# Hippogriff/parsenet-codebase

Measured on AMD Instinct MI355X. Metric: shapes/sec fwd+bwd on 10k-pt clouds, higher is better.
Workload: dtype f32; 1 GPU; cfg5: ParSeNet e2e (seg + mean-shift 10 it. + per-segment spline/primitive fit + Chamfer/residual), 10k pts, batch 4 per GPU, fwd+bwd+allreduce+Adam; batch_per_gpu=4, points=10000, k=80, parallelism=dp1, global_batch=4

## Files before the change

parsenet_codebase_amd/csrc/knn.hip:

```cpp
#include "knn_common.h"

__global__ void pn_knn_sqnorm_kernel(const float* __restrict__ x, int C, int N, int c0, int c1,
                                     float* __restrict__ xx, const int* __restrict__ gate_any) {
  const int b = blockIdx.y;
  if (gate_any && !gate_any[b]) return;
  const int j = blockIdx.x * blockDim.x + threadIdx.x;
  if (j >= N) return;
  const float* xb = x + (size_t)b * C * N;
  float acc = 0.f;
  for (int c = c0; c < c1; ++c) {
    float v = xb[(size_t)c * N + j];
    acc = __builtin_fmaf(v, v, acc);
  }
  xx[(size_t)b * N + j] = acc;
}

template <int MODE, bool TAIL>
__device__ static inline void knn_tile(const float* __restrict__ xb, const float* __restrict__ xxb,
                                       int C, int Nend, int j0, int qc, int N, float xxq,
                                       float tau, int& cnt, u64* __restrict__ mylist) {
  float acc[KNN_TC];
  float accn[MODE == 1 ? KNN_TC : 1];
#pragma unroll
  for (int t = 0; t < KNN_TC; ++t) acc[t] = 0.f;
// ... 43 lines not shown
    const bool ok = TAIL ? (j0 + t < Nend) : true;
    if (ok && v >= tau) {
      mylist[cnt] = knn_key(v, j0 + t);
      ++cnt;
    }
  }
}

template <int MODE>
__global__ __launch_bounds__(256) void pn_knn_scan_kernel(const float* __restrict__ x,
                                                          const float* __restrict__ xx, int C,
                                                          int N, int k, int S, int slice_len,
                                                          u64* __restrict__ lists,
                                                          int* __restrict__ counts,
                                                          KnnIdxOut out,
                                                          const int* __restrict__ gate) {
  __shared__ __attribute__((aligned(16))) uint32_t s_hist[4][256];
  const int b = blockIdx.z;
  const int slice = blockIdx.y;
  const int wave = threadIdx.x >> 6, lane = threadIdx.x & 63;
  const int qbase = (blockIdx.x * 4 + wave) * 64;
  if (qbase >= N) return;
  const int q = qbase + lane;
  const bool qvalid = q < N;
  const int qc = qvalid ? q : N - 1;
  const int Np = (N + 63) & ~63;
  if (gate && !__any(qvalid && gate[(size_t)b * N + qc] != 0)) return;
  const float* __restrict__ xb = x + (size_t)b * C * N;
  const float* __restrict__ xxb = xx + (size_t)b * N;
  u64* __restrict__ wlists = lists + (((size_t)b * Np + qbase) * S + slice) * KNN_CAP;
  const size_t lstride = (size_t)S * KNN_CAP;
  u64* __restrict__ mylist = wlists + (size_t)lane * lstride;
  uint32_t* hist = s_hist[wave];
// ... 98 lines not shown
  *slice_len_out = len;
}

size_t pn_knn_v1_workspace(int B, int C, int N, int k, bool gated) {
  (void)C;
  int S, len;
  knn_plan(B, N, k, gated, &S, &len);
  const size_t Np = pn_align_up(N, 64);
  return pn_align_up((size_t)B * N * sizeof(float), 256) +
         pn_align_up((size_t)B * Np * S * sizeof(int), 256) +
         pn_align_up((size_t)B * Np * S * KNN_CAP * sizeof(u64), 256);
}

int pn_knn_v1_launch(int mode, const float* x, int B, int C, int N, int k, KnnIdxOut idx,
                     void* workspace, size_t workspace_bytes, hipStream_t stream,
                     const int* gate, const int* gate_any) {
  PN_CHECK_ARG(x && idx.p, "pn_knn: null pointer");
  PN_CHECK_ARG(B > 0 && C > 0 && N > 0, "pn_knn: empty input (B=%d C=%d N=%d)", B, C, N);
  PN_CHECK_ARG(k >= 1 && k <= KNN_MAXK, "pn_knn: k=%d unsupported (1..%d)", k, KNN_MAXK);
  PN_CHECK_ARG(k <= N, "pn_knn: k=%d exceeds the number of points N=%d", k, N);
  PN_CHECK_ARG(mode == 0 || C == 6, "pn_knn_pn: points+normals metric needs C=6, got %d", C);
  PN_CHECK_ARG(workspace && workspace_bytes >= pn_knn_v1_workspace(B, C, N, k, gate != nullptr),
               "pn_knn: workspace too small");
  int S, slice_len;
  knn_plan(B, N, k, gate != nullptr, &S, &slice_len);
  const size_t Np = pn_align_up(N, 64);
  char* w = (char*)workspace;
  float* xx = (float*)w;
  w += pn_align_up((size_t)B * N * sizeof(float), 256);
  int* counts = (int*)w;
  w += pn_align_up((size_t)B * Np * S * sizeof(int), 256);
  u64* lists = (u64*)w;
  dim3 g1(pn_cdiv(N, 256), B);
  hipLaunchKernelGGL(pn_knn_sqnorm_kernel, g1, dim3(256), 0, stream, x, C, N, 0,
                     mode == 0 ? C : 3, xx, gate ? gate_any : nullptr);
  PN_CHECK_LAUNCH();
  dim3 grid(pn_cdiv(N, 256), S, B);
  PN_PROF(gate ? "knn_scan_gated" : "knn_scan", stream);
  if (mode == 0)
    hipLaunchKernelGGL(pn_knn_scan_kernel<0>, grid, dim3(256), 0, stream, x, xx, C, N, k, S,
                       slice_len, lists, counts, idx, gate);
  else
    hipLaunchKernelGGL(pn_knn_scan_kernel<1>, grid, dim3(256), 0, stream, x, xx, C, N, k, S,
                       slice_len, lists, counts, idx, gate);
  PN_CHECK_LAUNCH();
  if (S > 1) {
    const long long nq = (long long)B * N;
    hipLaunchKernelGGL(pn_knn_merge_kernel, dim3(pn_cdiv(nq, 4)), dim3(256), 0, stream, lists,
                       counts, N, k, S, nq, idx);
    PN_CHECK_LAUNCH();
  }
  return PN_OK;
}
```

parsenet_codebase_amd/csrc/knn_common.h:

```cpp
#pragma once
#include "common.h"

#define KNN_TC 32
#define KNN_CAP 1024
#define KNN_CAP0 256
#define KNN_MAXK 128
#define KNN_EPL (KNN_CAP / 64)

typedef unsigned long long u64;

struct KnnIdxOut {
  void* p;
  int is32;
  __host__ __device__ explicit operator bool() const { return p != nullptr; }
  __device__ inline void put(size_t pos, int64_t v) const {
    if (is32)
      static_cast<int*>(p)[pos] = (int)v;
    else
      static_cast<int64_t*>(p)[pos] = v;
  }
};

__device__ static inline u64 knn_key(float v, int j) {
  if (v == 0.0f) v = 0.0f;
  return ((u64)pn_f2ord(v) << 32) | (u64)(0xffffffffu - (uint32_t)j);
}
__device__ static inline int64_t knn_key_index(u64 key) {
  return key ? (int64_t)(0xffffffffu - (uint32_t)(key & 0xffffffffu)) : 0;
}

__device__ static inline u64 readlane_u64(u64 v, int l) {
  uint32_t lo = __builtin_amdgcn_readlane((uint32_t)v, l);
  uint32_t hi = __builtin_amdgcn_readlane((uint32_t)(v >> 32), l);
  return ((u64)hi << 32) | lo;
}

__device__ static u64 knn_wave_select_ge(u64* __restrict__ lp, int n, int k, uint32_t* __restrict__ hist,
                                         float slack, int* __restrict__ kept) {
  const int lane = threadIdx.x & 63;
  u64 key[KNN_EPL];
#pragma unroll
  for (int e = 0; e < KNN_EPL; ++e) {
    int s = e * 64 + lane;
// ... 113 lines not shown
```

parsenet_codebase_amd/csrc/knn_mfma.hip:

```cpp
#include "knn_common.h"
#include "split_common.h"

typedef float f32x16 __attribute__((ext_vector_type(16)));

size_t pn_knn_v1_workspace(int B, int C, int N, int k, bool gated);
int pn_knn_v1_launch(int mode, const float* x, int B, int C, int N, int k, KnnIdxOut idx,
                     void* workspace, size_t workspace_bytes, hipStream_t stream,
                     const int* gate, const int* gate_any = nullptr);

struct KnnPerm {
  uint32_t a, c, mask;
  int n;
};

__host__ __device__ static inline int knn_perm(const KnnPerm& p, int i) {
  uint32_t v = (uint32_t)i;
  do {
    v = (v * p.a + p.c) & p.mask;
  } while (v >= (uint32_t)p.n);
  return (int)v;
}

static KnnPerm knn_make_perm(int N, bool identity) {
  KnnPerm p;
  int m = 1;
  while ((1u << m) < (uint32_t)N) ++m;
  p.mask = (m >= 32) ? 0xffffffffu : ((1u << m) - 1u);
  p.a = identity ? 1u : (((uint32_t)(0.6180339887498949 * (double)(1ull << m))) | 1u);
  p.c = identity ? 0u : ((0x9E3779B9u >> (32 - m)) | 1u);
  p.n = N;
  return p;
}

__global__ void pn_knn_prep_kernel(const float* __restrict__ x, int C, int N, int Cp, int Np,
                                   int mode, int point_major, KnnPerm perm,
                                   float* __restrict__ xp, float* __restrict__ xxp) {
  const int b = blockIdx.y;
  const int jp = blockIdx.x * blockDim.x + threadIdx.x;
  if (jp >= Np) return;
  const float* xb = x + (size_t)b * C * N;
  float* xpb = xp + (size_t)b * Cp * Np;
  float acc = 0.f;
  if (jp < N) {
    const int j = knn_perm(perm, jp);
    const int cnorm = mode == 1 ? 3 : C;
    int c = 0;
    for (; c + 8 <= C; c += 8) {
      float v[8];
#pragma unroll
      for (int e = 0; e < 8; ++e) v[e] = point_major ? xb[(size_t)j * C + c + e] : xb[(size_t)(c + e) * N + j];
#pragma unroll
      for (int e = 0; e < 8; ++e) {
        const int cd = (mode == 1 && c + e >= 3) ? c + e + 1 : c + e;
        xpb[(size_t)cd * Np + jp] = v[e];
        if (c + e < cnorm) acc = __builtin_fmaf(v[e], v[e], acc);
      }
    }
    for (; c < C; ++c) {
      const float v = point_major ? xb[(size_t)j * C + c] : xb[(size_t)c * N + j];
      const int cd = (mode == 1 && c >= 3) ? c + 1 : c;
      xpb[(size_t)cd * Np + jp] = v;
      if (c < cnorm) acc = __builtin_fmaf(v, v, acc);
    }
    if (mode == 1) {
      xpb[(size_t)3 * Np + jp] = 0.f;
      xpb[(size_t)7 * Np + jp] = 0.f;
    } else {
      for (int c = C; c < Cp; ++c) xpb[(size_t)c * Np + jp] = 0.f;
    }
  } else {
    for (int c = 0; c < Cp; ++c) xpb[(size_t)c * Np + jp] = 0.f;
  }
  xxp[(size_t)b * Np + jp] = acc;
}

__global__ __launch_bounds__(256) void pn_knn_prep_pm_kernel(const float* __restrict__ x, int C, int N,
                                                            int Cp, int Np, KnnPerm perm,
                                                            float* __restrict__ xp,
                                                            float* __restrict__ xxp) {
  extern __shared__ float prep_tile[];
  const int b = blockIdx.y;
  const int jp0 = blockIdx.x * 64;
  const int t = threadIdx.x;
  const float* xb = x + (size_t)b * C * N;
// ... 13 lines not shown
  const int p = t & 63, part = t >> 6;
  if (jp0 + p < Np) {
    for (int c = part; c < Cp; c += 4) xpb[(size_t)c * Np + jp0 + p] = c < C ? prep_tile[p * ld + c] : 0.f;
    if (part == 0) {
      float acc = 0.f;
      for (int c = 0; c < C; ++c) {
        const float v = prep_tile[p * ld + c];
        acc = __builtin_fmaf(v, v, acc);
      }
      xxp[(size_t)b * Np + jp0 + p] = acc;
    }
  }
}

static void knn_prep_launch(hipStream_t stream, const float* x, int B, int C, int N, int Cp, int Np, int mode,
                            int point_major, KnnPerm perm, float* xp, float* xxp) {
  if (point_major && mode != 1 && (C & 3) == 0 && C <= 224) {
    hipLaunchKernelGGL(pn_knn_prep_pm_kernel, dim3(pn_cdiv(Np, 64), B), dim3(256), 64 * (C + 1) * sizeof(float),
                       stream, x, C, N, Cp, Np, perm, xp, xxp);
  } else {
    hipLaunchKernelGGL(pn_knn_prep_kernel, dim3(pn_cdiv(Np, 64), B), dim3(64), 0, stream, x, C, N, Cp, Np,
                       mode, point_major, perm, xp, xxp);
  }
}

template <int KSTEPS, int QSETS, int MODE, int KIND>
__global__ __launch_bounds__(256) void pn_knn_mfma_kernel(
    const float* __restrict__ xq, const float* __restrict__ xxq_, int Nq, int Nqp,
    const float* __restrict__ xc, const float* __restrict__ xxc_, int Nc, int Ncp,
    int tiles_per_slice, float* __restrict__ tilemax, const float* __restrict__ tau,
    u64* __restrict__ lists, int* __restrict__ counts, int subcap, KnnPerm perm_c) {
  constexpr bool COLLECT = KIND == 1;
  constexpr bool ARGMAX = KIND == 2;
  constexpr int CP = 2 * KSTEPS;
  constexpr int TILE = CP * 32;
  __shared__ __attribute__((aligned(16))) float lds[2][TILE + 32];
  const int b = blockIdx.z;
// ... 153 lines not shown

__global__ void pn_knn_argmax_final_kernel(const u64* __restrict__ lists, int Nq, int Nqp, int S,
                                           KnnPerm perm_q, KnnIdxOut out_idx) {
  const int b = blockIdx.y;
  const int qp = blockIdx.x * blockDim.x + threadIdx.x;
  if (qp >= Nq) return;
  const u64* l = lists + ((size_t)b * Nqp + qp) * S * 2;
  u64 best = 0;
  for (int i = 0; i < 2 * S; ++i) best = l[i] > best ? l[i] : best;
  out_idx.put((size_t)b * Nq + knn_perm(perm_q, qp), knn_key_index(best));
}

#define KM_TR 16
__global__ __launch_bounds__(256) void pn_knn_tau_kernel(const float* __restrict__ tilemax, int Nq,
                                                         int Nqp, int T, int k,
                                                         float* __restrict__ tau) {
  const int b = blockIdx.y;
  const int wave = threadIdx.x >> 6, lane = threadIdx.x & 63;
  const int q = blockIdx.x * 4 + wave;
  if (q >= Nq) return;
  const float* __restrict__ row = tilemax + ((size_t)b * Nqp + q) * T;
  float v[KM_TR];
  float vmin = __builtin_inff(), vmax = -__builtin_inff();
#pragma unroll
  for (int e = 0; e < KM_TR; ++e) {
    const int t = e * 64 + lane;
    v[e] = t < T ? row[t] : -__builtin_inff();
    if (v[e] > -__builtin_inff()) vmin = fminf(vmin, v[e]);
    vmax = fmaxf(vmax, v[e]);
  }
  for (int t = KM_TR * 64 + lane; t < T; t += 64) {
// ... 14 lines not shown
    const float fm = pn_ord2f(mid);
    int c = 0;
#pragma unroll
    for (int e = 0; e < KM_TR; ++e) c += __builtin_popcountll(__ballot(v[e] >= fm));
    for (int t0 = KM_TR * 64; t0 < T; t0 += 64) {
      const int t = t0 + lane;
      c += __builtin_popcountll(__ballot(t < T && row[t] >= fm));
    }
    if (c >= k) {
      lo = mid;
      if (c <= k + slack) break;
    } else {
      hi = mid;
    }
  }
  if (lane == 0) tau[(size_t)b * Nqp + q] = pn_ord2f(lo);
}

__global__ __launch_bounds__(256) void pn_knn_final_kernel(
    const u64* __restrict__ lists, const int* __restrict__ counts, int Nq, int Nqp, int k, int S,
    int subcap, KnnPerm perm_q, KnnPerm perm_c, KnnIdxOut out_idx,
    float* __restrict__ out_val, int* __restrict__ flags, int* __restrict__ anyflag) {
  __shared__ __attribute__((aligned(16))) uint32_t s_hist[4][256];
  __shared__ u64 s_keys[4][KNN_CAP];
  const int b = blockIdx.y;
  const int wave = threadIdx.x >> 6, lane = threadIdx.x & 63;
  const int qp = blockIdx.x * 4 + wave;
  if (qp >= Nq) return;
  const size_t ql = (size_t)b * Nqp + qp;
  const int qo = knn_perm(perm_q, qp);
  u64* keys = s_keys[wave];
  const int nsub = 2 * S;
// ... 202 lines not shown
  if (kind == 0)
    hipLaunchKernelGGL((pn_knn_mfma_kernel<KSTEPS, QSETS, MODE, 0>), grid, dim3(256), 0, stream, xq,
                       xxq, Nq, Nqp, xc, xxc, Nc, Ncp, tps, tilemax, tau, lists, cnt, subcap, perm_c);
  else if (kind == 1)
    hipLaunchKernelGGL((pn_knn_mfma_kernel<KSTEPS, QSETS, MODE, 1>), grid, dim3(256), 0, stream, xq,
                       xxq, Nq, Nqp, xc, xxc, Nc, Ncp, tps, tilemax, tau, lists, cnt, subcap, perm_c);
  else if (MODE == 2)
    hipLaunchKernelGGL((pn_knn_mfma_kernel<KSTEPS, QSETS, MODE, (MODE == 2 ? 2 : 0)>), grid,
                       dim3(256), 0, stream, xq, xxq, Nq, Nqp, xc, xxc, Nc, Ncp, tps, tilemax, tau,
                       lists, cnt, subcap, perm_c);
}

static int select_run(const KnnPlan& p, const KnnWs& w, int mode, bool self, const float* q,
                      int q_pm, int Nq, const float* c, int c_pm, int Nc, int B, int C, int k,
                      KnnIdxOut out_idx, float* out_val, int* flags_out, char* base,
                      hipStream_t stream, bool approx_value = false) {
  float* xc = (float*)(base + w.xc);
  float* xxc = (float*)(base + w.xxc);
  float* xq = (float*)(base + w.xq);
  float* xxq = (float*)(base + w.xxq);
  float* tilemax = (float*)(base + w.tilemax);
  float* tau = (float*)(base + w.tau);
  int* cnt = (int*)(base + w.cnt);
  int* flags = flags_out ? flags_out : (int*)(base + w.flags);
  int* anyflag = flags_out ? nullptr : flags + (size_t)B * Nq;
  u64* lists = (u64*)(base + w.lists);
  const bool argmax = mode == 2 && k == 1 && out_val == nullptr && out_idx.p != nullptr && !self;
  const KnnPerm perm_c = knn_make_perm(Nc, argmax);
  const KnnPerm perm_q = self ? perm_c : knn_make_perm(Nq, true);

  PN_CHECK_HIP(hipMemsetAsync(flags, 0, ((size_t)B * Nq + (flags_out ? 0 : B)) * 4, stream));
  {
    PN_PROF("knn_prep", stream);
    knn_prep_launch(stream, c, B, C, Nc, p.Cp, p.Ncp, mode, c_pm, perm_c, xc, xxc);
    if (!self) knn_prep_launch(stream, q, B, C, Nq, p.Cp, p.Nqp, mode, q_pm, perm_q, xq, xxq);
  }
  PN_CHECK_LAUNCH();
  const bool x3p1 = !argmax && (approx_value ? knn_x3_pass1(p, 0, true) : knn_x3_pass1(p, mode));
  if (approx_value && !(x3p1 && mode == 2 && out_val && !out_idx.p)) {
    pn_set_error("select_run: the bf16 x 3 value selection needs C <= 128 and Nc >= 2048");
    return PN_ERR_UNSUPPORTED;
  }
  const bool x3p2 = x3p1 && knn_x3_level() >= 2 && self && mode == 0 && out_idx.p && !out_val;
  u32x4* img = (u32x4*)(base + w.img);
  unsigned* xxmax = (unsigned*)(base + w.xxmax);
  float* xpm = x3p2 ? (float*)(base + w.xpm) : nullptr;
  float* xxo = x3p2 ? (float*)(base + w.xxo) : nullptr;
  const float x3A = 4.0f * (float)(p.Cp + 2) * 0x1p-24f;
  const bool centre = x3p2 && knn_x3_centre();
  const float x3Ao = centre ? (float)(p.Cp + 4) * 0x1p-24f : 0.f;
  const int np1 = knn_x3_p1_products(mode, centre);
  const float x3A1 = np1 == 3 ? x3A + 3.1f * 0x1p-16f : x3A;
  const int np2 = (centre && np1 == 3 && getenv("PN_KNN_X3_P2") && atoi(getenv("PN_KNN_X3_P2")) == 3) ? 3 : 6;
  const float x3A2 = np2 == 3 ? x3A1 : x3A;
  float* mu = centre ? (float*)(base + w.mu) : nullptr;
  float* xpc = centre ? (float*)(base + w.xpc) : nullptr;
  float* xxcc = centre ? (float*)(base + w.xxcc) : nullptr;
  float* xxoc = centre ? (float*)(base + w.xxoc) : nullptr;
  unsigned* xxmaxc = centre ? (unsigned*)(base + w.xxmaxc) : nullptr;
  if (x3p1) {
    PN_PROF("knn_x3_image", stream);
    PN_CHECK_HIP(hipMemsetAsync(xxmax, 0, (size_t)B * 8, stream));
    if (centre) {
      hipLaunchKernelGGL(pn_knn_x3_mean_kernel, dim3(p.Cp, B), dim3(256), 0, stream, (const float*)xc, p.Cp, p.Ncp, Nc, mu);
    }
    dim3 ig(p.Ncp / 32, B);
    if (p.ksteps == 32)
      hipLaunchKernelGGL(pn_knn_x3_image_kernel<8>, ig, dim3(256), 0, stream, xc, xxc, p.Ncp, img, xxmax, Nc, perm_c,
                         xpm, xxo, (const float*)mu, xpc, xxcc, xxoc, xxmaxc);
    else if (p.ksteps == 64)
      hipLaunchKernelGGL(pn_knn_x3_image_kernel<16>, ig, dim3(256), 0, stream, xc, xxc, p.Ncp, img, xxmax, Nc, perm_c,
                         xpm, xxo, (const float*)mu, xpc, xxcc, xxoc, xxmaxc);
    else
      hipLaunchKernelGGL(pn_knn_x3_image_kernel<32>, ig, dim3(256), 0, stream, xc, xxc, p.Ncp, img, xxmax, Nc, perm_c,
                         xpm, xxo, (const float*)mu, xpc, xxcc, xxoc, xxmaxc);
    PN_CHECK_LAUNCH();
  }
  const float* xq_a = centre ? (const float*)xpc : (const float*)xq;
  const float* xxq_a = centre ? (const float*)xxcc : (const float*)xxq;
  const float* xxc_a = centre ? (const float*)xxcc : (const float*)xxc;
  const unsigned* xxmax_a = centre ? (const unsigned*)xxmaxc : (const unsigned*)xxmax;
  if (p.fused && x3p2) {
    const char* ne = getenv("PN_KNN_FUSED_NP");
    const int npf = (ne && atoi(ne) == 6) ? 6 : 3;
    const float Af = npf == 3 ? x3A + 3.1f * 0x1p-16f : x3A;
    const int qpw = 128 * p.qsets, ntiles = p.Ncp / 32, subcapf = KNN_CAP / 2;
    dim3 gf(1, pn_cdiv(p.Nqp, qpw), B);
    {
      PN_PROF(p.ksteps == 32 ? "knn_x3_fused_c64" : "knn_x3_fused_wide", stream);
#define KX_GOF(NCH, QS, TPS_, NP_)                                                                                       \
// ... 60 lines not shown
  }
        if (mode == 0 && p.ksteps == 32)
          KX_GO1(8, 2, 0, 2)
        else if (mode == 0 && p.ksteps == 64)
          KX_GO1(16, 1, 0, 1)
        else if (mode == 0)
          KX_GO1(32, 1, 0, 1)
        else if (p.ksteps == 32)
          KX_GO1(8, 2, 2, 2)
        else
          KX_GO1(16, 1, 2, 1)
      }
      PN_CHECK_LAUNCH();
      {
        PN_PROF("knn_tau", stream);
        hipLaunchKernelGGL(pn_knn_tau_kernel, dim3(pn_cdiv(Nq, 4), B), dim3(256), 0, stream,
                           tilemax, Nq, p.Nqp, p.Ncp / 16, k, tau);
        if (!approx_value || np1 == 3)
          hipLaunchKernelGGL(pn_knn_x3_margin_kernel, dim3(pn_cdiv(Nq, 256), B), dim3(256), 0, stream, tau, xxq_a, Nq,
                             p.Nqp, xxmax_a, x3p2 ? x3A2 : x3A, mode, (x3p2 || approx_value) ? 2.0f : 1.0f, x3A1,
                             (const float*)xxq, (const unsigned*)xxmax, x3Ao);
      }
      PN_CHECK_LAUNCH();
      if (approx_value) {
        int tpsv = tps1;
        if (pn_cdiv(ntiles, tpsv) > KX_MAX_SLICES) tpsv = (int)pn_align_up(pn_cdiv(ntiles, KX_MAX_SLICES), 2);
        const int Sv = pn_cdiv(ntiles, tpsv);
        int subcapv = (int)pn_align_up(3 * k / (2 * Sv) + 16, 8);
        if (2 * Sv * subcapv > 2 * p.S * p.subcap) subcapv = (2 * p.S * p.subcap) / (2 * Sv);
        if (2 * Sv * subcapv > KNN_CAP) subcapv = KNN_CAP / (2 * Sv);
        dim3 gv(Sv, pn_cdiv(p.Nqp, qpw), B);
        {
          PN_PROF("sel_x3_pass2_dot", stream);
          if (p.ksteps == 32)
            KX_GO(8, 2, 2, 2, 1, gv, tpsv, subcapv);
          else
// ... 82 lines not shown
        KM_GO(2, 2, 0);
      else if (p.ksteps == 4)
        KM_GO(4, 2, 0);
      else if (p.ksteps == 32)
        KM_GO(32, 2, 0);
      else if (p.ksteps == 64)
        KM_GO(64, 1, 0);
      else
        KM_GO(128, 1, 0);
#undef KM_GO
    }
    PN_CHECK_LAUNCH();
    if (collect == 0) {
      PN_PROF("knn_tau", stream);
      hipLaunchKernelGGL(pn_knn_tau_kernel, dim3(pn_cdiv(Nq, 4), B), dim3(256), 0, stream,
                         tilemax, Nq, p.Nqp, p.Ncp / 16, k, tau);
      PN_CHECK_LAUNCH();
    }
  }
  if (argmax) {
    PN_PROF("knn_final", stream);
    hipLaunchKernelGGL(pn_knn_argmax_final_kernel, dim3(pn_cdiv(Nq, 256), B), dim3(256), 0, stream, lists,
                       Nq, p.Nqp, p.S, perm_q, out_idx);
    PN_CHECK_LAUNCH();
    return PN_OK;
  }
  {
    PN_PROF("knn_final", stream);
    hipLaunchKernelGGL(pn_knn_final_kernel, dim3(pn_cdiv(Nq, 4), B), dim3(256), 0, stream, lists,
                       cnt, Nq, p.Nqp, k, p.S, p.subcap, perm_q, perm_c, out_idx, out_val, flags, anyflag);
  }
// ... 145 lines not shown
  const int tps = pn_cdiv(ntiles, S);
  S = pn_cdiv(ntiles, tps);
  int subcap = (int)pn_align_up(3 * k / (2 * S) + 16, 8);
  if (2 * S * subcap > 2 * p.S * p.subcap) subcap = (2 * p.S * p.subcap) / (2 * S);
  if (2 * S * subcap > KNN_CAP) subcap = KNN_CAP / (2 * S);
  dim3 grid(S, pn_cdiv(Nq, 256), B);
  {
    PN_PROF("sel_h2_pass1_dot", stream);
    hipLaunchKernelGGL(pn_dotsel_h2_kernel<0>, grid, dim3(512), 0, stream, q, Nq, p.Nqp, (const u32x4*)img_c,
                       Nc, p.Ncp, tps, tilemax, (const float*)tau, lists, cnt, subcap);
  }
  PN_CHECK_LAUNCH();
  {
    PN_PROF("knn_tau", stream);
    hipLaunchKernelGGL(pn_knn_tau_kernel, dim3(pn_cdiv(Nq, 4), B), dim3(256), 0, stream, tilemax, Nq, p.Nqp,
                       p.Ncp / 16, k, tau);
  }
  PN_CHECK_LAUNCH();
  {
    PN_PROF("sel_h2_pass2_dot", stream);
    hipLaunchKernelGGL(pn_dotsel_h2_kernel<1>, grid, dim3(512), 0, stream, q, Nq, p.Nqp, (const u32x4*)img_c,
                       Nc, p.Ncp, tps, tilemax, (const float*)tau, lists, cnt, subcap);
  }
  PN_CHECK_LAUNCH();
  {
    PN_PROF("knn_final", stream);
    hipLaunchKernelGGL(pn_knn_final_kernel, dim3(pn_cdiv(Nq, 4), B), dim3(256), 0, stream, lists, cnt, Nq,
                       p.Nqp, k, S, subcap, ident_q, ident_c, KnnIdxOut{nullptr, 0}, out_val, flags, (int*)nullptr);
  }
  PN_CHECK_LAUNCH();
  return PN_OK;
// ... 24 lines not shown
  PN_CHECK_ARG(k >= 1 && k <= KNN_MAXK, "pn_knn: k=%d unsupported (1..%d)", k, KNN_MAXK);
  PN_CHECK_ARG(k <= N, "pn_knn: k=%d exceeds the number of points N=%d", k, N);
  PN_CHECK_ARG(mode == 0 || C == 6, "pn_knn_pn: points+normals metric needs C=6, got %d", C);
  PN_CHECK_ARG(workspace && workspace_bytes >= pn_knn_workspace(B, C, N, k),
               "pn_knn: workspace too small");
  const KnnPlan p = knn_mfma_plan(mode, B, C, N, N, k, false);
  if (!(p.fused && knn_x3_level() >= 2)) {
    const KskPlan sk = ksk_plan(mode, B, C, N, k);
    if (sk.ok) return ksk_run(sk, x, B, C, N, k, idx.p, idx.is32, (char*)workspace, stream);
  }
  if (!p.fast)
    return pn_knn_v1_launch(mode, x, B, C, N, k, idx, workspace, workspace_bytes, stream, nullptr);
  const KnnWs w = knn_mfma_ws(p, B, C, N, k, true, true);
  char* base = (char*)workspace;
  int rc = select_run(p, w, mode, true, x, 0, N, x, 0, N, B, C, k, idx, nullptr, nullptr, base,
                      stream);
  if (rc) return rc;
  PN_PROF("knn_fallback_gate", stream);
  return pn_knn_v1_launch(mode, x, B, C, N, k, idx, base + w.v1,
                          pn_knn_v1_workspace(B, C, N, k, true), stream, (int*)(base + w.flags),
                          (int*)(base + w.flags) + (size_t)B * N);
}

extern "C" int pn_knn_f32(const float* x, int B, int C, int N, int k, int64_t* idx,
                          void* workspace, size_t workspace_bytes, void* stream) {
  return knn_dispatch(0, x, B, C, N, k, KnnIdxOut{idx, 0}, workspace, workspace_bytes, (hipStream_t)stream);
}

extern "C" int pn_knn_pn_f32(const float* x6, int B, int N, int k, int64_t* idx, void* workspace,
                             size_t workspace_bytes, void* stream) {
  return knn_dispatch(1, x6, B, 6, N, k, KnnIdxOut{idx, 0}, workspace, workspace_bytes, (hipStream_t)stream);
}

extern "C" int pn_knn_graph_i32(const float* x, int B, int C, int N, int k, int metric, int32_t* idx,
                                void* workspace, size_t workspace_bytes, void* stream) {
  PN_CHECK_ARG(metric == 0 || metric == 1, "pn_knn_graph_i32: metric %d", metric);
// ... 28 lines not shown
```

parsenet_codebase_amd/csrc/knn_x3.h:

```cpp
#pragma once

template <int NCH>
__host__ __device__ static inline int knx_slot(int r, int q) {
  return r * NCH + (q ^ (NCH == 8 ? ((r >> 1) & 7) : x3_swz(r)));
}

__global__ __launch_bounds__(256) void pn_knn_x3_mean_kernel(const float* __restrict__ xp, int CP, int Np, int N,
                                                             float* __restrict__ mu) {
  __shared__ float red[256];
  const int c = blockIdx.x, b = blockIdx.y, t = threadIdx.x;
  const float* row = xp + ((size_t)b * CP + c) * Np;
  float acc = 0.f;
  for (int j = t; j < N; j += 256) acc += row[j];
  red[t] = acc;
  __syncthreads();
#pragma unroll
  for (int o = 128; o > 0; o >>= 1) {
    if (t < o) red[t] += red[t + o];
    __syncthreads();
  }
  if (t == 0) mu[(size_t)b * CP + c] = red[0] / (float)N;
}

template <int NCH>
__global__ __launch_bounds__(256) void pn_knn_x3_image_kernel(const float* __restrict__ xp,
                                                              const float* __restrict__ xxp, int Np,
                                                              u32x4* __restrict__ img,
                                                              unsigned* __restrict__ xxmax, int N, KnnPerm perm,
                                                              float* __restrict__ xpm, float* __restrict__ xxo,
                                                              const float* __restrict__ mu, float* __restrict__ xpc,
                                                              float* __restrict__ xxcc, float* __restrict__ xxoc,
                                                              unsigned* __restrict__ xxmaxc) {
  constexpr int CP = 8 * NCH;
  __shared__ double s_part[8][32][2];
  const int b = blockIdx.y, t = blockIdx.x, tid = threadIdx.x;
  const int r = tid & 31;
  const float* src = xp + (size_t)b * CP * Np + (size_t)t * 32 + r;
  u32x4* dst = img + ((size_t)b * (Np / 32) + t) * (3 * 32 * NCH);
  const int jp = t * 32 + r;
  const int jo = (xpm && jp < N) ? knn_perm(perm, jp) : -1;
  double part_mx = 0.0, part_mm = 0.0;
  for (int q = tid >> 5; q < NCH; q += 8) {
    float v[8];
#pragma unroll
    for (int e = 0; e < 8; ++e) v[e] = src[(size_t)(8 * q + e) * Np];
    if (jo >= 0) {
      float4* d = reinterpret_cast<float4*>(xpm + ((size_t)b * N + jo) * CP + 8 * q);
      d[0] = make_float4(v[0], v[1], v[2], v[3]);
      d[1] = make_float4(v[4], v[5], v[6], v[7]);
    }
    if (mu) {
#pragma unroll
      for (int e = 0; e < 8; ++e) {
        const float m = mu[(size_t)b * CP + 8 * q + e];
        part_mx = __builtin_fma((double)m, (double)v[e], part_mx);
        part_mm = __builtin_fma((double)m, (double)m, part_mm);
        v[e] = jp < N ? v[e] - m : 0.f;
        xpc[((size_t)b * CP + 8 * q + e) * Np + jp] = v[e];
      }
    }
    u32x4 vh, vm, vl;
    X3_SPLIT_TO(v[0], v[1], vh, vm, vl, 0);
    X3_SPLIT_TO(v[2], v[3], vh, vm, vl, 1);
    X3_SPLIT_TO(v[4], v[5], vh, vm, vl, 2);
    X3_SPLIT_TO(v[6], v[7], vh, vm, vl, 3);
    const int slot = knx_slot<NCH>(r, q);
    dst[slot] = vh;
    dst[32 * NCH + slot] = vm;
    dst[2 * 32 * NCH + slot] = vl;
  }
  if (mu) {
    s_part[tid >> 5][r][0] = part_mx;
    s_part[tid >> 5][r][1] = part_mm;
    __syncthreads();
  }
  if (tid < 64) {
    const float nrm = tid < 32 ? xxp[(size_t)b * Np + (size_t)t * 32 + tid] : 0.f;
    if (tid < 32 && jo >= 0) xxo[(size_t)b * N + jo] = nrm;
    const float m = pn_wave_max(nrm);
    if (tid == 0) atomicMax(&xxmax[b], __float_as_uint(fmaxf(m, 0.f)));
    if (mu) {
      float nc = 0.f;
      if (tid < 32) {
        double mx = 0.0, mm = 0.0;
#pragma unroll
        for (int g = 0; g < 8; ++g) {
          mx += s_part[g][tid][0];
          mm += s_part[g][tid][1];
        }
        nc = jp < N ? (float)(((double)nrm - 2.0 * mx) + mm) : 0.f;
        xxcc[(size_t)b * Np + (size_t)t * 32 + tid] = nc;
        if (jo >= 0) xxoc[(size_t)b * N + jo] = nc;
      }
      const float mc = pn_wave_max(nc);
      if (tid == 0) atomicMax(&xxmaxc[b], __float_as_uint(fmaxf(mc, 0.f)));
    }
  }
}

__device__ static inline float knx_eps(float nq, float nc, float A, int mode) {
  nq = fmaxf(nq, 0.f);
  nc = fmaxf(nc, 0.f);
  const float cross = sqrtf(nq * nc) * 1.000001f;
  return (mode == 0 ? 2.0f * A * cross + 0x1p-21f * (nq + nc) : A * cross) * 1.0001f;
}

#define KX_NW 4
#define KX_WPE(NCH, MODE) ((NCH) == 32 ? 1 : ((NCH) == 16 && (MODE) == 2 ? 3 : 2))
template <int NCH, int QSETS, int MODE, int TPS, int KIND, int NP = 6>
__global__ __launch_bounds__(64 * KX_NW) __attribute__((amdgpu_waves_per_eu(KX_WPE(NCH, MODE), KX_WPE(NCH, MODE)))) void pn_knn_x3_pass_kernel(
    const float* __restrict__ xq, const float* __restrict__ xxq_, int Nq, int Nqp,
    const u32x4* __restrict__ PC, const float* __restrict__ xxc_, int Nc, int Ncp, int tiles_per_slice,
    float* __restrict__ tilemax, const float* __restrict__ tau, u64* __restrict__ lists,
    int* __restrict__ counts, int subcap, const unsigned* __restrict__ xxmax,
    const float* __restrict__ xxq_o = nullptr, const unsigned* __restrict__ xxmax_o = nullptr, float A_ = 0.f,
    float Ao_ = 0.f) {
  static_assert(KIND != 2 || MODE == 0, "the fused form is built for the squared-distance metric");
  constexpr int CP = 8 * NCH, KS = NCH / 2, PIECE = 32 * NCH, IMG = 3 * PIECE;
  constexpr int CHUNKS = TPS * IMG / 64;
  static_assert(CHUNKS % KX_NW == 0 && (TPS == 1 || TPS == 2 || TPS == 4), "chunks are dealt evenly to the waves");
// ... 241 lines not shown
      }
    }
    cur ^= 1;
  }
#undef KX_STAGE
  if (KIND >= 1 && wave_on) {
#pragma unroll
    for (int u = 0; u < QSETS; ++u) {
      const int q = q0 + 32 * u + col;
      if (q < Nqp) counts[(((size_t)b * Nqp + q) * gridDim.x + slice) * 2 + h] = mycnt[u];
    }
  }
}


__global__ void pn_knn_x3_margin_kernel(float* __restrict__ tau, const float* __restrict__ xxq, int Nq, int Nqp,
                                        const unsigned* __restrict__ xxmax, float A, int mode, float times, float A1,
                                        const float* __restrict__ xxq_o, const unsigned* __restrict__ xxmax_o, float Ao) {
  const int b = blockIdx.y;
  const int q = blockIdx.x * blockDim.x + threadIdx.x;
  if (q >= Nq) return;
  const float nq = xxq[(size_t)b * Nqp + q], nc = __uint_as_float(xxmax[b]);
  float eps = knx_eps(nq, nc, A1, mode) + (times - 1.0f) * knx_eps(nq, nc, A, mode);
  if (Ao > 0.f) eps += times * knx_eps(xxq_o[(size_t)b * Nqp + q], __uint_as_float(xxmax_o[b]), Ao, mode);
  const float t = tau[(size_t)b * Nqp + q];
  tau[(size_t)b * Nqp + q] = t - eps - 0x1p-22f * fabsf(t);
}

template <int CP>
__device__ static inline float knx_exact_dot(const float* __restrict__ xq, const float* __restrict__ xcrow) {
  constexpr int CB = CP > 128 ? 128 : CP;
  float dot = 0.f;
#pragma clang loop unroll(disable)
  for (int c0 = 0; c0 < CP; c0 += CB) {
    const float4* xc = reinterpret_cast<const float4*>(xcrow + c0);
    float4 cv[CB / 4];
#pragma unroll
    for (int c4 = 0; c4 < CB / 4; ++c4) cv[c4] = xc[c4];
#pragma unroll
    for (int c4 = 0; c4 < CB / 4; ++c4) {
      const float4 qv = *reinterpret_cast<const float4*>(xq + c0 + 4 * c4);
      dot = __builtin_fmaf(qv.x, cv[c4].x, dot);
      dot = __builtin_fmaf(qv.y, cv[c4].y, dot);
// ... 145 lines not shown
```

Baseline: 178.5 shapes/s.

## Fuse KNN prep, mean, margin and flag-clear kernels; reuse norms in fallback

Merges several small KNN launches. The centred x3 path now reads the source directly in a combined mean and prep kernel, and zeroing of flags and maxima moves into the prep kernels, which drops memsets. The tau margin is folded into the tau kernel. The v1 fallback reuses squared norms written by prep and exits early for batches with no gated points. This trims launch and memory-pass overhead, but the new prep kernel recomputes norms from shared memory and reads strided source data, and the fallback's correctness now depends on xx being written in prep.

Result: no change. 178.0 shapes/s (-0.3%).

```diff
diff --git a/parsenet_codebase_amd/csrc/knn.hip b/parsenet_codebase_amd/csrc/knn.hip
--- a/parsenet_codebase_amd/csrc/knn.hip
+++ b/parsenet_codebase_amd/csrc/knn.hip
@@ -81,9 +81,11 @@
                                                           u64* __restrict__ lists,
                                                           int* __restrict__ counts,
                                                           KnnIdxOut out,
-                                                          const int* __restrict__ gate) {
+                                                          const int* __restrict__ gate,
+                                                          const int* __restrict__ gate_any) {
   __shared__ __attribute__((aligned(16))) uint32_t s_hist[4][256];
   const int b = blockIdx.z;
+  if (gate_any && !gate_any[b]) return;
   const int slice = blockIdx.y;
   const int wave = threadIdx.x >> 6, lane = threadIdx.x & 63;
   const int qbase = (blockIdx.x * 4 + wave) * 64;
@@ -212,7 +214,7 @@
 
 int pn_knn_v1_launch(int mode, const float* x, int B, int C, int N, int k, KnnIdxOut idx,
                      void* workspace, size_t workspace_bytes, hipStream_t stream,
-                     const int* gate, const int* gate_any) {
+                     const int* gate, const int* gate_any, bool xx_ready) {
   PN_CHECK_ARG(x && idx.p, "pn_knn: null pointer");
   PN_CHECK_ARG(B > 0 && C > 0 && N > 0, "pn_knn: empty input (B=%d C=%d N=%d)", B, C, N);
   PN_CHECK_ARG(k >= 1 && k <= KNN_MAXK, "pn_knn: k=%d unsupported (1..%d)", k, KNN_MAXK);
@@ -229,18 +231,20 @@
   int* counts = (int*)w;
   w += pn_align_up((size_t)B * Np * S * sizeof(int), 256);
   u64* lists = (u64*)w;
-  dim3 g1(pn_cdiv(N, 256), B);
-  hipLaunchKernelGGL(pn_knn_sqnorm_kernel, g1, dim3(256), 0, stream, x, C, N, 0,
-                     mode == 0 ? C : 3, xx, gate ? gate_any : nullptr);
-  PN_CHECK_LAUNCH();
+  if (!xx_ready) {
+    dim3 g1(pn_cdiv(N, 256), B);
+    hipLaunchKernelGGL(pn_knn_sqnorm_kernel, g1, dim3(256), 0, stream, x, C, N, 0,
+                       mode == 0 ? C : 3, xx, gate ? gate_any : nullptr);
+    PN_CHECK_LAUNCH();
+  }
   dim3 grid(pn_cdiv(N, 256), S, B);
   PN_PROF(gate ? "knn_scan_gated" : "knn_scan", stream);
   if (mode == 0)
     hipLaunchKernelGGL(pn_knn_scan_kernel<0>, grid, dim3(256), 0, stream, x, xx, C, N, k, S,
-                       slice_len, lists, counts, idx, gate);
+                       slice_len, lists, counts, idx, gate, gate ? gate_any : nullptr);
   else
     hipLaunchKernelGGL(pn_knn_scan_kernel<1>, grid, dim3(256), 0, stream, x, xx, C, N, k, S,
-                       slice_len, lists, counts, idx, gate);
+                       slice_len, lists, counts, idx, gate, gate ? gate_any : nullptr);
   PN_CHECK_LAUNCH();
   if (S > 1) {
     const long long nq = (long long)B * N;
diff --git a/parsenet_codebase_amd/csrc/knn_common.h b/parsenet_codebase_amd/csrc/knn_common.h
--- a/parsenet_codebase_amd/csrc/knn_common.h
+++ b/parsenet_codebase_amd/csrc/knn_common.h
@@ -27,6 +27,30 @@
 }
 __device__ static inline int64_t knn_key_index(u64 key) {
   return key ? (int64_t)(0xffffffffu - (uint32_t)(key & 0xffffffffu)) : 0;
+}
+
+__device__ static inline float knx_eps(float nq, float nc, float A, int mode) {
+  nq = fmaxf(nq, 0.f);
+  nc = fmaxf(nc, 0.f);
+  const float cross = sqrtf(nq * nc) * 1.000001f;
+  return (mode == 0 ? 2.0f * A * cross + 0x1p-21f * (nq + nc) : A * cross) * 1.0001f;
+}
+
+struct KnxMargin {
+  const float* xxq;
+  const unsigned* xxmax;
+  float A;
+  int mode;
+  float times, A1;
+  const float* xxq_o;
+  const unsigned* xxmax_o;
+  float Ao;
+};
+__device__ static inline float knx_lower(const KnxMargin& g, float t, int b, size_t qi) {
+  const float nq = g.xxq[qi], nc = __uint_as_float(g.xxmax[b]);
+  float eps = knx_eps(nq, nc, g.A1, g.mode) + (g.times - 1.0f) * knx_eps(nq, nc, g.A, g.mode);
+  if (g.Ao > 0.f) eps += g.times * knx_eps(g.xxq_o[qi], __uint_as_float(g.xxmax_o[b]), g.Ao, g.mode);
+  return t - eps - 0x1p-22f * fabsf(t);
 }
 
 __device__ static inline u64 readlane_u64(u64 v, int l) {
diff --git a/parsenet_codebase_amd/csrc/knn_mfma.hip b/parsenet_codebase_amd/csrc/knn_mfma.hip
--- a/parsenet_codebase_amd/csrc/knn_mfma.hip
+++ b/parsenet_codebase_amd/csrc/knn_mfma.hip
@@ -6,7 +6,7 @@
 size_t pn_knn_v1_workspace(int B, int C, int N, int k, bool gated);
 int pn_knn_v1_launch(int mode, const float* x, int B, int C, int N, int k, KnnIdxOut idx,
                      void* workspace, size_t workspace_bytes, hipStream_t stream,
-                     const int* gate, const int* gate_any = nullptr);
+                     const int* gate, const int* gate_any = nullptr, bool xx_ready = false);
 
 struct KnnPerm {
   uint32_t a, c, mask;
@@ -34,10 +34,14 @@
 
 __global__ void pn_knn_prep_kernel(const float* __restrict__ x, int C, int N, int Cp, int Np,
                                    int mode, int point_major, KnnPerm perm,
-                                   float* __restrict__ xp, float* __restrict__ xxp) {
+                                   float* __restrict__ xp, float* __restrict__ xxp,
+                                   float* __restrict__ xxo, int* __restrict__ flags,
+                                   int* __restrict__ anyflag) {
   const int b = blockIdx.y;
   const int jp = blockIdx.x * blockDim.x + threadIdx.x;
   if (jp >= Np) return;
+  if (flags && jp < N) flags[(size_t)b * N + jp] = 0;
+  if (anyflag && jp == 0) anyflag[b] = 0;
   const float* xb = x + (size_t)b * C * N;
   float* xpb = xp + (size_t)b * Cp * Np;
   float acc = 0.f;
@@ -68,6 +72,7 @@
     } else {
       for (int c = C; c < Cp; ++c) xpb[(size_t)c * Np + jp] = 0.f;
     }
+    if (xxo) xxo[(size_t)b * N + j] = acc;
   } else {
     for (int c = 0; c < Cp; ++c) xpb[(size_t)c * Np + jp] = 0.f;
   }
@@ -111,13 +116,14 @@
 }
 
 static void knn_prep_launch(hipStream_t stream, const float* x, int B, int C, int N, int Cp, int Np, int mode,
-                            int point_major, KnnPerm perm, float* xp, float* xxp) {
-  if (point_major && mode != 1 && (C & 3) == 0 && C <= 224) {
+                            int point_major, KnnPerm perm, float* xp, float* xxp, float* xxo = nullptr,
+                            int* flags = nullptr, int* anyflag = nullptr) {
+  if (!xxo && !flags && point_major && mode != 1 && (C & 3) == 0 && C <= 224) {
     hipLaunchKernelGGL(pn_knn_prep_pm_kernel, dim3(pn_cdiv(Np, 64), B), dim3(256), 64 * (C + 1) * sizeof(float),
                        stream, x, C, N, Cp, Np, perm, xp, xxp);
   } else {
     hipLaunchKernelGGL(pn_knn_prep_kernel, dim3(pn_cdiv(Np, 64), B), dim3(64), 0, stream, x, C, N, Cp, Np,
-                       mode, point_major, perm, xp, xxp);
+                       mode, point_major, perm, xp, xxp, xxo, flags, anyflag);
   }
 }
 
@@ -301,7 +307,7 @@
 #define KM_TR 16
 __global__ __launch_bounds__(256) void pn_knn_tau_kernel(const float* __restrict__ tilemax, int Nq,
                                                          int Nqp, int T, int k,
-                                                         float* __restrict__ tau) {
+                                                         float* __restrict__ tau, KnxMargin margin) {
   const int b = blockIdx.y;
   const int wave = threadIdx.x >> 6, lane = threadIdx.x & 63;
   const int q = blockIdx.x * 4 + wave;
@@ -346,8 +352,12 @@
       hi = mid;
     }
   }
-  if (lane == 0) tau[(size_t)b * Nqp + q] = pn_ord2f(lo);
-}
+  if (lane == 0) {
+    const float t = pn_ord2f(lo);
+    tau[(size_t)b * Nqp + q] = margin.xxq ? knx_lower(margin, t, b, (size_t)b * Nqp + q) : t;
+  }
+}
+static const KnxMargin knx_no_margin = {nullptr, nullptr, 0.f, 0, 1.0f, 0.f, nullptr, nullptr, 0.f};
 
 __global__ __launch_bounds__(256) void pn_knn_final_kernel(
     const u64* __restrict__ lists, const int* __restrict__ counts, int Nq, int Nqp, int k, int S,
@@ -580,7 +590,7 @@
 static int select_run(const KnnPlan& p, const KnnWs& w, int mode, bool self, const float* q,
                       int q_pm, int Nq, const float* c, int c_pm, int Nc, int B, int C, int k,
                       KnnIdxOut out_idx, float* out_val, int* flags_out, char* base,
-                      hipStream_t stream, bool approx_value = false) {
+                      hipStream_t stream, bool approx_value = false, float* xx_orig = nullptr) {
   float* xc = (float*)(base + w.xc);
   float* xxc = (float*)(base + w.xxc);
   float* xq = (float*)(base + w.xq);
@@ -595,25 +605,29 @@
   const KnnPerm perm_c = knn_make_perm(Nc, argmax);
   const KnnPerm perm_q = self ? perm_c : knn_make_perm(Nq, true);
 
-  PN_CHECK_HIP(hipMemsetAsync(flags, 0, ((size_t)B * Nq + (flags_out ? 0 : B)) * 4, stream));
-  {
-    PN_PROF("knn_prep", stream);
-    knn_prep_launch(stream, c, B, C, Nc, p.Cp, p.Ncp, mode, c_pm, perm_c, xc, xxc);
-    if (!self) knn_prep_launch(stream, q, B, C, Nq, p.Cp, p.Nqp, mode, q_pm, perm_q, xq, xxq);
-  }
-  PN_CHECK_LAUNCH();
   const bool x3p1 = !argmax && (approx_value ? knn_x3_pass1(p, 0, true) : knn_x3_pass1(p, mode));
   if (approx_value && !(x3p1 && mode == 2 && out_val && !out_idx.p)) {
     pn_set_error("select_run: the bf16 x 3 value selection needs C <= 128 and Nc >= 2048");
     return PN_ERR_UNSUPPORTED;
   }
   const bool x3p2 = x3p1 && knn_x3_level() >= 2 && self && mode == 0 && out_idx.p && !out_val;
+  const bool centre = x3p2 && knn_x3_centre();
   u32x4* img = (u32x4*)(base + w.img);
   unsigned* xxmax = (unsigned*)(base + w.xxmax);
   float* xpm = x3p2 ? (float*)(base + w.xpm) : nullptr;
-  float* xxo = x3p2 ? (float*)(base + w.xxo) : nullptr;
+  float* xxo = (self && xx_orig) ? xx_orig : (x3p2 ? (float*)(base + w.xxo) : nullptr);
+  if (!self) PN_CHECK_HIP(hipMemsetAsync(flags, 0, ((size_t)B * Nq + (flags_out ? 0 : B)) * 4, stream));
+  if (!centre) {
+    PN_PROF("knn_prep", stream);
+    if (self) {
+      knn_prep_launch(stream, c, B, C, Nc, p.Cp, p.Ncp, mode, c_pm, perm_c, xc, xxc, xx_orig, flags, anyflag);
+    } else {
+      knn_prep_launch(stream, c, B, C, Nc, p.Cp, p.Ncp, mode, c_pm, perm_c, xc, xxc);
+      knn_prep_launch(stream, q, B, C, Nq, p.Cp, p.Nqp, mode, q_pm, perm_q, xq, xxq);
+    }
+  }
+  PN_CHECK_LAUNCH();
   const float x3A = 4.0f * (float)(p.Cp + 2) * 0x1p-24f;
-  const bool centre = x3p2 && knn_x3_centre();
   const float x3Ao = centre ? (float)(p.Cp + 4) * 0x1p-24f : 0.f;
   const int np1 = knn_x3_p1_products(mode, centre);
   const float x3A1 = np1 == 3 ? x3A + 3.1f * 0x1p-16f : x3A;
@@ -624,22 +638,35 @@
   float* xxcc = centre ? (float*)(base + w.xxcc) : nullptr;
   float* xxoc = centre ? (float*)(base + w.xxoc) : nullptr;
   unsigned* xxmaxc = centre ? (unsigned*)(base + w.xxmaxc) : nullptr;
-  if (x3p1) {
+  if (centre) {
+    PN_PROF("knn_prep_x3", stream);
+    hipLaunchKernelGGL(pn_knn_x3_mean_src_kernel, dim3(p.Cp, B), dim3(256), 0, stream, c, C, p.Cp, Nc, c_pm, perm_c, mu,
+                       xxmax, xxmaxc);
+    dim3 ig(p.Ncp / 32, B);
+#define KX_PREP(NCH)                                                                                                \
+  hipLaunchKernelGGL(pn_knn_x3_prep_kernel<NCH>, ig, dim3(256), 0, stream, c, C, Nc, p.Ncp, c_pm, perm_c,           \
+                     (const float*)mu, img, xpm, xxo, xxc, xpc, xxcc, xxoc, xxmax, xxmaxc, flags, anyflag)
+    if (p.ksteps == 32)
+      KX_PREP(8);
+    else if (p.ksteps == 64)
+      KX_PREP(16);
+    else
+      KX_PREP(32);
+#undef KX_PREP
+    PN_CHECK_LAUNCH();
+  } else if (x3p1) {
     PN_PROF("knn_x3_image", stream);
-    PN_CHECK_HIP(hipMemsetAsync(xxmax, 0, (size_t)B * 8, stream));
-    if (centre) {
-      hipLaunchKernelGGL(pn_knn_x3_mean_kernel, dim3(p.Cp, B), dim3(256), 0, stream, (const float*)xc, p.Cp, p.Ncp, Nc, mu);
-    }
+    PN_CHECK_HIP(hipMemsetAsync(xxmax, 0, (size_t)B * 4, stream));
     dim3 ig(p.Ncp / 32, B);
     if (p.ksteps == 32)
       hipLaunchKernelGGL(pn_knn_x3_image_kernel<8>, ig, dim3(256), 0, stream, xc, xxc, p.Ncp, img, xxmax, Nc, perm_c,
-                         xpm, xxo, (const float*)mu, xpc, xxcc, xxoc, xxmaxc);
+                         xpm, xxo);
     else if (p.ksteps == 64)
       hipLaunchKernelGGL(pn_knn_x3_image_kernel<16>, ig, dim3(256), 0, stream, xc, xxc, p.Ncp, img, xxmax, Nc, perm_c,
-                         xpm, xxo, (const float*)mu, xpc, xxcc, xxoc, xxmaxc);
+                         xpm, xxo);
     else
       hipLaunchKernelGGL(pn_knn_x3_image_kernel<32>, ig, dim3(256), 0, stream, xc, xxc, p.Ncp, img, xxmax, Nc, perm_c,
-                         xpm, xxo, (const float*)mu, xpc, xxcc, xxoc, xxmaxc);
+                         xpm, xxo);
     PN_CHECK_LAUNCH();
   }
   const float* xq_a = centre ? (const float*)xpc : (const float*)xq;
@@ -730,12 +757,10 @@
       PN_CHECK_LAUNCH();
       {
         PN_PROF("knn_tau", stream);
-        hipLaunchKernelGGL(pn_knn_tau_kernel, dim3(pn_cdiv(Nq, 4), B), dim3(256), 0, stream,
-                           tilemax, Nq, p.Nqp, p.Ncp / 16, k, tau);
-        if (!approx_value || np1 == 3)
-          hipLaunchKernelGGL(pn_knn_x3_margin_kernel, dim3(pn_cdiv(Nq, 256), B), dim3(256), 0, stream, tau, xxq_a, Nq,
-                             p.Nqp, xxmax_a, x3p2 ? x3A2 : x3A, mode, (x3p2 || approx_value) ? 2.0f : 1.0f, x3A1,
-                             (const float*)xxq, (const unsigned*)xxmax, x3Ao);
+        const KnxMargin mg = {xxq_a, xxmax_a, x3p2 ? x3A2 : x3A, mode, (x3p2 || approx_value) ? 2.0f : 1.0f, x3A1,
+                              (const float*)xxq, (const unsigned*)xxmax, x3Ao};
+        hipLaunchKernelGGL(pn_knn_tau_kernel, dim3(pn_cdiv(Nq, 4), B), dim3(256), 0, stream, tilemax, Nq, p.Nqp,
+                           p.Ncp / 16, k, tau, (!approx_value || np1 == 3) ? mg : knx_no_margin);
       }
       PN_CHECK_LAUNCH();
       if (approx_value) {
@@ -848,7 +873,7 @@
     if (collect == 0) {
       PN_PROF("knn_tau", stream);
       hipLaunchKernelGGL(pn_knn_tau_kernel, dim3(pn_cdiv(Nq, 4), B), dim3(256), 0, stream,
-                         tilemax, Nq, p.Nqp, p.Ncp / 16, k, tau);
+                         tilemax, Nq, p.Nqp, p.Ncp / 16, k, tau, knx_no_margin);
       PN_CHECK_LAUNCH();
     }
   }
@@ -1024,7 +1049,7 @@
   {
     PN_PROF("knn_tau", stream);
     hipLaunchKernelGGL(pn_knn_tau_kernel, dim3(pn_cdiv(Nq, 4), B), dim3(256), 0, stream, tilemax, Nq, p.Nqp,
-                       p.Ncp / 16, k, tau);
+                       p.Ncp / 16, k, tau, knx_no_margin);
   }
   PN_CHECK_LAUNCH();
   {
@@ -1079,12 +1104,11 @@
   const KnnWs w = knn_mfma_ws(p, B, C, N, k, true, true);
   char* base = (char*)workspace;
   int rc = select_run(p, w, mode, true, x, 0, N, x, 0, N, B, C, k, idx, nullptr, nullptr, base,
-                      stream);
+                      stream, false, (float*)(base + w.v1));
   if (rc) return rc;
-  PN_PROF("knn_fallback_gate", stream);
   return pn_knn_v1_launch(mode, x, B, C, N, k, idx, base + w.v1,
                           pn_knn_v1_workspace(B, C, N, k, true), stream, (int*)(base + w.flags),
-                          (int*)(base + w.flags) + (size_t)B * N);
+                          (int*)(base + w.flags) + (size_t)B * N, true);
 }
 
 extern "C" int pn_knn_f32(const float* x, int B, int C, int N, int k, int64_t* idx,
diff --git a/parsenet_codebase_amd/csrc/knn_x3.h b/parsenet_codebase_amd/csrc/knn_x3.h
--- a/parsenet_codebase_amd/csrc/knn_x3.h
+++ b/parsenet_codebase_amd/csrc/knn_x3.h
@@ -3,23 +3,6 @@
 template <int NCH>
 __host__ __device__ static inline int knx_slot(int r, int q) {
   return r * NCH + (q ^ (NCH == 8 ? ((r >> 1) & 7) : x3_swz(r)));
-}
-
-__global__ __launch_bounds__(256) void pn_knn_x3_mean_kernel(const float* __restrict__ xp, int CP, int Np, int N,
-                                                             float* __restrict__ mu) {
-  __shared__ float red[256];
-  const int c = blockIdx.x, b = blockIdx.y, t = threadIdx.x;
-  const float* row = xp + ((size_t)b * CP + c) * Np;
-  float acc = 0.f;
-  for (int j = t; j < N; j += 256) acc += row[j];
-  red[t] = acc;
-  __syncthreads();
-#pragma unroll
-  for (int o = 128; o > 0; o >>= 1) {
-    if (t < o) red[t] += red[t + o];
-    __syncthreads();
-  }
-  if (t == 0) mu[(size_t)b * CP + c] = red[0] / (float)N;
 }
 
 template <int NCH>
@@ -27,19 +10,14 @@
                                                               const float* __restrict__ xxp, int Np,
                                                               u32x4* __restrict__ img,
                                                               unsigned* __restrict__ xxmax, int N, KnnPerm perm,
-                                                              float* __restrict__ xpm, float* __restrict__ xxo,
-                                                              const float* __restrict__ mu, float* __restrict__ xpc,
-                                                              float* __restrict__ xxcc, float* __restrict__ xxoc,
-                                                              unsigned* __restrict__ xxmaxc) {
+                                                              float* __restrict__ xpm, float* __restrict__ xxo) {
   constexpr int CP = 8 * NCH;
-  __shared__ double s_part[8][32][2];
   const int b = blockIdx.y, t = blockIdx.x, tid = threadIdx.x;
   const int r = tid & 31;
   const float* src = xp + (size_t)b * CP * Np + (size_t)t * 32 + r;
   u32x4* dst = img + ((size_t)b * (Np / 32) + t) * (3 * 32 * NCH);
   const int jp = t * 32 + r;
   const int jo = (xpm && jp < N) ? knn_perm(perm, jp) : -1;
-  double part_mx = 0.0, part_mm = 0.0;
   for (int q = tid >> 5; q < NCH; q += 8) {
     float v[8];
 #pragma unroll
@@ -48,16 +26,6 @@
       float4* d = reinterpret_cast<float4*>(xpm + ((size_t)b * N + jo) * CP + 8 * q);
       d[0] = make_float4(v[0], v[1], v[2], v[3]);
       d[1] = make_float4(v[4], v[5], v[6], v[7]);
-    }
-    if (mu) {
-#pragma unroll
-      for (int e = 0; e < 8; ++e) {
-        const float m = mu[(size_t)b * CP + 8 * q + e];
-        part_mx = __builtin_fma((double)m, (double)v[e], part_mx);
-        part_mm = __builtin_fma((double)m, (double)m, part_mm);
-        v[e] = jp < N ? v[e] - m : 0.f;
-        xpc[((size_t)b * CP + 8 * q + e) * Np + jp] = v[e];
-      }
     }
     u32x4 vh, vm, vl;
     X3_SPLIT_TO(v[0], v[1], vh, vm, vl, 0);
@@ -69,41 +37,127 @@
     dst[32 * NCH + slot] = vm;
     dst[2 * 32 * NCH + slot] = vl;
   }
-  if (mu) {
-    s_part[tid >> 5][r][0] = part_mx;
-    s_part[tid >> 5][r][1] = part_mm;
-    __syncthreads();
-  }
   if (tid < 64) {
     const float nrm = tid < 32 ? xxp[(size_t)b * Np + (size_t)t * 32 + tid] : 0.f;
     if (tid < 32 && jo >= 0) xxo[(size_t)b * N + jo] = nrm;
     const float m = pn_wave_max(nrm);
     if (tid == 0) atomicMax(&xxmax[b], __float_as_uint(fmaxf(m, 0.f)));
-    if (mu) {
-      float nc = 0.f;
-      if (tid < 32) {
-        double mx = 0.0, mm = 0.0;
-#pragma unroll
-        for (int g = 0; g < 8; ++g) {
-          mx += s_part[g][tid][0];
-          mm += s_part[g][tid][1];
-        }
-        nc = jp < N ? (float)(((double)nrm - 2.0 * mx) + mm) : 0.f;
-        xxcc[(size_t)b * Np + (size_t)t * 32 + tid] = nc;
-        if (jo >= 0) xxoc[(size_t)b * N + jo] = nc;
-      }
-      const float mc = pn_wave_max(nc);
-      if (tid == 0) atomicMax(&xxmaxc[b], __float_as_uint(fmaxf(mc, 0.f)));
-    }
-  }
-}
-
-__device__ static inline float knx_eps(float nq, float nc, float A, int mode) {
-  nq = fmaxf(nq, 0.f);
-  nc = fmaxf(nc, 0.f);
-  const float cross = sqrtf(nq * nc) * 1.000001f;
-  return (mode == 0 ? 2.0f * A * cross + 0x1p-21f * (nq + nc) : A * cross) * 1.0001f;
-}
+  }
+}
+
+
+__global__ __launch_bounds__(256) void pn_knn_x3_mean_src_kernel(const float* __restrict__ x, int C, int CP, int N,
+                                                                 int point_major, KnnPerm perm, float* __restrict__ mu,
+                                                                 unsigned* __restrict__ xxmax,
+                                                                 unsigned* __restrict__ xxmaxc) {
+  __shared__ float red[256];
+  const int c = blockIdx.x, b = blockIdx.y, t = threadIdx.x;
+  if (c == 0 && t == 0) {
+    xxmax[b] = 0u;
+    xxmaxc[b] = 0u;
+  }
+  if (c >= C) {
+    if (t == 0) mu[(size_t)b * CP + c] = 0.f;
+    return;
+  }
+  const float* xb = x + (size_t)b * C * N;
+  float acc = 0.f;
+  for (int j = t; j < N; j += 256) {
+    const int jo = knn_perm(perm, j);
+    acc += point_major ? xb[(size_t)jo * C + c] : xb[(size_t)c * N + jo];
+  }
+  red[t] = acc;
+  __syncthreads();
+#pragma unroll
+  for (int o = 128; o > 0; o >>= 1) {
+    if (t < o) red[t] += red[t + o];
+    __syncthreads();
+  }
+  if (t == 0) mu[(size_t)b * CP + c] = red[0] / (float)N;
+}
+
+template <int NCH>
+__global__ __launch_bounds__(256) void pn_knn_x3_prep_kernel(const float* __restrict__ x, int C, int N, int Np,
+                                                             int point_major, KnnPerm perm,
+                                                             const float* __restrict__ mu, u32x4* __restrict__ img,
+                                                             float* __restrict__ xpm, float* __restrict__ xxo,
+                                                             float* __restrict__ xxp, float* __restrict__ xpc,
+                                                             float* __restrict__ xxcc, float* __restrict__ xxoc,
+                                                             unsigned* __restrict__ xxmax,
+                                                             unsigned* __restrict__ xxmaxc, int* __restrict__ flags,
+                                                             int* __restrict__ anyflag) {
+  constexpr int CP = 8 * NCH;
+  __shared__ float s_x[CP][33];
+  __shared__ double s_part[8][32][2];
+  const int b = blockIdx.y, t = blockIdx.x, tid = threadIdx.x;
+  const int r = tid & 31;
+  const float* xb = x + (size_t)b * C * N;
+  u32x4* dst = img + ((size_t)b * (Np / 32) + t) * (3 * 32 * NCH);
+  const int jp = t * 32 + r;
+  const int jo = jp < N ? knn_perm(perm, jp) : -1;
+  if (tid < 32 && jp < N) flags[(size_t)b * N + jp] = 0;
+  if (anyflag && t == 0 && tid == 0) anyflag[b] = 0;
+  double part_mx = 0.0, part_mm = 0.0;
+  for (int q = tid >> 5; q < NCH; q += 8) {
+    float v[8];
+#pragma unroll
+    for (int e = 0; e < 8; ++e) {
+      const int c = 8 * q + e;
+      v[e] = (jo >= 0 && c < C) ? (point_major ? xb[(size_t)jo * C + c] : xb[(size_t)c * N + jo]) : 0.f;
+      s_x[c][r] = v[e];
+    }
+    if (jo >= 0) {
+      float4* d = reinterpret_cast<float4*>(xpm + ((size_t)b * N + jo) * CP + 8 * q);
+      d[0] = make_float4(v[0], v[1], v[2], v[3]);
+      d[1] = make_float4(v[4], v[5], v[6], v[7]);
+    }
+#pragma unroll
+    for (int e = 0; e < 8; ++e) {
+      const float m = mu[(size_t)b * CP + 8 * q + e];
+      part_mx = __builtin_fma((double)m, (double)v[e], part_mx);
+      part_mm = __builtin_fma((double)m, (double)m, part_mm);
+      v[e] = jp < N ? v[e] - m : 0.f;
+      xpc[((size_t)b * CP + 8 * q + e) * Np + jp] = v[e];
+    }
+    u32x4 vh, vm, vl;
+    X3_SPLIT_TO(v[0], v[1], vh, vm, vl, 0);
+    X3_SPLIT_TO(v[2], v[3], vh, vm, vl, 1);
+    X3_SPLIT_TO(v[4], v[5], vh, vm, vl, 2);
+    X3_SPLIT_TO(v[6], v[7], vh, vm, vl, 3);
+    const int slot = knx_slot<NCH>(r, q);
+    dst[slot] = vh;
+    dst[32 * NCH + slot] = vm;
+    dst[2 * 32 * NCH + slot] = vl;
+  }
+  s_part[tid >> 5][r][0] = part_mx;
+  s_part[tid >> 5][r][1] = part_mm;
+  __syncthreads();
+  if (tid < 64) {
+    float nrm = 0.f;
+    if (tid < 32 && jo >= 0) {
+      for (int c = 0; c < C; ++c) nrm = __builtin_fmaf(s_x[c][tid], s_x[c][tid], nrm);
+      xxo[(size_t)b * N + jo] = nrm;
+    }
+    if (tid < 32) xxp[(size_t)b * Np + jp] = nrm;
+    const float m = pn_wave_max(nrm);
+    if (tid == 0) atomicMax(&xxmax[b], __float_as_uint(fmaxf(m, 0.f)));
+    float nc = 0.f;
+    if (tid < 32) {
+      double mx = 0.0, mm = 0.0;
+#pragma unroll
+      for (int g = 0; g < 8; ++g) {
+        mx += s_part[g][tid][0];
+        mm += s_part[g][tid][1];
+      }
+      nc = jp < N ? (float)(((double)nrm - 2.0 * mx) + mm) : 0.f;
+      xxcc[(size_t)b * Np + jp] = nc;
+      if (jo >= 0) xxoc[(size_t)b * N + jo] = nc;
+    }
+    const float mc = pn_wave_max(nc);
+    if (tid == 0) atomicMax(&xxmaxc[b], __float_as_uint(fmaxf(mc, 0.f)));
+  }
+}
+
 
 #define KX_NW 4
 #define KX_WPE(NCH, MODE) ((NCH) == 32 ? 1 : ((NCH) == 16 && (MODE) == 2 ? 3 : 2))
@@ -375,19 +429,6 @@
 }
 
 
-__global__ void pn_knn_x3_margin_kernel(float* __restrict__ tau, const float* __restrict__ xxq, int Nq, int Nqp,
-                                        const unsigned* __restrict__ xxmax, float A, int mode, float times, float A1,
-                                        const float* __restrict__ xxq_o, const unsigned* __restrict__ xxmax_o, float Ao) {
-  const int b = blockIdx.y;
-  const int q = blockIdx.x * blockDim.x + threadIdx.x;
-  if (q >= Nq) return;
-  const float nq = xxq[(size_t)b * Nqp + q], nc = __uint_as_float(xxmax[b]);
-  float eps = knx_eps(nq, nc, A1, mode) + (times - 1.0f) * knx_eps(nq, nc, A, mode);
-  if (Ao > 0.f) eps += times * knx_eps(xxq_o[(size_t)b * Nqp + q], __uint_as_float(xxmax_o[b]), Ao, mode);
-  const float t = tau[(size_t)b * Nqp + q];
-  tau[(size_t)b * Nqp + q] = t - eps - 0x1p-22f * fabsf(t);
-}
-
 template <int CP>
 __device__ static inline float knx_exact_dot(const float* __restrict__ xq, const float* __restrict__ xcrow) {
   constexpr int CB = CP > 128 ? 128 : CP;
```
